# luxfi/tfhe

Hardware: AMD Instinct MI355X
Metric: PBS/sec at TFHE 128-bit default (N=1024), batch=4096; 1/2/4/8 MI355X (higher is better)
Workload: dtype f64

## Files before the change

tfhe_amd/csrc/pbs_fft.hip:

```cpp
#pragma clang fp contract(off)
#include <hip/hip_runtime.h>

#include <type_traits>

#include "fft512.h"
#include "gl64.h"
#include "ntt1024.h"
#include "pbs_kernels.h"

namespace tfhe {
namespace fftk {

__device__ __forceinline__ void fft_fwd_real(const double (&a)[16], double (&xr)[8], double (&xi)[8], double2* T,
                                             int lane, const double2* tw) {
#pragma unroll
  for (int e = 0; e < 8; e++) {
    xr[e] = a[e];
    xi[e] = a[e + 8];
  }
  dft512_fwd(xr, xi, T, lane, TBase(lane), tw);
}

__device__ __forceinline__ void fft_inv_real(double (&xr)[8], double (&xi)[8], double2* T, int lane, TBase tb,
                                             const double2* tw) {
  dft512_inv(xr, xi, T, lane, tb, tw);
  twist_slots<true>(xr, xi);
}

__device__ __forceinline__ int ms2048(u64 x) { return (int)((((x >> 52) + 1) >> 1) & 2047u); }

__device__ __forceinline__ u32 decomp_state(u64 x) { return ((u32)(x >> 32) + 1024u) >> 11; }
__device__ __forceinline__ int decomp_step(u32& st, u32 bmask) {
  const u32 b = __builtin_amdgcn_ubfe(st, 13, bmask);
  const u32 W = st + 63u + b;
  const u32 stn = W >> 7;
  int d;
  asm("v_mad_i32_i24 %0, %1, %2, %3" : "=v"(d) : "v"(stn), "s"(-128), "v"(st));
  st = stn;
  return d;
}
__device__ __forceinline__ u32 decomp_state_not(u64 S) { return (1023u - (u32)(S >> 32)) >> 11; }
__device__ __forceinline__ double decomp_top(u32 st) {
  int t;
  asm("v_bfe_i32 %0, %1, 0, 7" : "=v"(t) : "v"(0u - st));
  return -(double)t;
}

__device__ __forceinline__ void mac_first(double& re, double& im, double dr, double di, double2 k) {
  re = dr * k.x;
  re = __builtin_fma(-di, k.y, re);
  im = dr * k.y;
  im = __builtin_fma(di, k.x, im);
}
__device__ __forceinline__ void mac_next(double& re, double& im, double dr, double di, double2 k) {
  re = __builtin_fma(dr, k.x, re);
  re = __builtin_fma(-di, k.y, re);
  im = __builtin_fma(dr, k.y, im);
  im = __builtin_fma(di, k.x, im);
}

constexpr double BSK_SCALE = 0x1p-41;
__global__ __launch_bounds__(64) void bsk_to_fourier_kernel(const u64* __restrict__ bsk_std,
                                                            double2* __restrict__ bsk_f,
                                                            const double2* __restrict__ tw) {
  __shared__ __attribute__((aligned(16))) double2 T[T_C64];
  const int lane = threadIdx.x;
  const size_t q = blockIdx.x;
  const u64* src = bsk_std + q * N1K;
  double a[16], xr[8], xi[8];
#pragma unroll
  for (int e = 0; e < 16; e++) a[e] = i64_to_f64(src[64 * e + lane]);
  fft_fwd_real(a, xr, xi, T, lane, tw);
  const size_t j = q % 2, r = (q / 2) % 6, i = q / 12;
  double2* dst = bsk_f + ((i * 6 + (r / 3) * 3 + (2 - r % 3)) * 2 + j) * M;
#pragma unroll
  for (int e = 0; e < 8; e++) dst[64 * e + lane] = make_double2(xr[e] * BSK_SCALE, xi[e] * BSK_SCALE);
}

__global__ __launch_bounds__(64) void fft_fwd_kernel(const u64* __restrict__ in, double2* __restrict__ out,
                                                     const double2* __restrict__ tw) {
  __shared__ __attribute__((aligned(16))) double2 T[T_C64];
  const int lane = threadIdx.x;
  const u64* src = in + (size_t)blockIdx.x * N1K;
  double a[16], xr[8], xi[8];
#pragma unroll
  for (int e = 0; e < 16; e++) a[e] = i64_to_f64(src[64 * e + lane]);
  fft_fwd_real(a, xr, xi, T, lane, tw);
  double2* dst = out + (size_t)blockIdx.x * M;
#pragma unroll
  for (int e = 0; e < 8; e++) dst[64 * e + lane] = make_double2(xr[e], xi[e]);
}

__global__ __launch_bounds__(64) void fft_inv_kernel(const double2* __restrict__ in, double* __restrict__ out,
                                                     const double2* __restrict__ tw) {
  __shared__ __attribute__((aligned(16))) double2 T[T_C64];
  const int lane = threadIdx.x;
  const double2* src = in + (size_t)blockIdx.x * M;
  double xr[8], xi[8];
#pragma unroll
  for (int e = 0; e < 8; e++) {
    const double2 v = src[64 * e + lane];
    xr[e] = v.x;
    xi[e] = v.y;
  }
  fft_inv_real(xr, xi, T, lane, TBase(lane), tw);
  double* dst = out + (size_t)blockIdx.x * N1K;
#pragma unroll
  for (int e = 0; e < 8; e++) {
    dst[64 * e + lane] = xr[e];
    dst[64 * (e + 8) + lane] = xi[e];
  }
}

constexpr unsigned dispatch_half(unsigned wg, unsigned cus) { return wg / cus; }
constexpr bool wg_prio_hi(unsigned wg, unsigned cus) { return dispatch_half(wg, cus) & 1u; }
constexpr bool wg_staggered(unsigned wg, unsigned cus) { return dispatch_half(wg, cus) == 1u; }
namespace dh_check {
constexpr bool same_as_bit8(unsigned n) {
  for (unsigned w = 0; w < n; w++)
    if (wg_prio_hi(w, 256) != (((w >> 8) & 1u) != 0) || wg_staggered(w, 256) != (w < 512 && ((w >> 8) & 1u))) return false;
  return true;
}
static_assert(same_as_bit8(4096), "dispatch_half(., 256) must reproduce the 256-CU split");
static_assert(!wg_prio_hi(31, 32) && wg_prio_hi(32, 32) && wg_prio_hi(63, 32) && !wg_prio_hi(64, 32) && wg_prio_hi(96, 32), "32 CUs");
static_assert(!wg_staggered(31, 32) && wg_staggered(32, 32) && wg_staggered(63, 32) && !wg_staggered(64, 32) && !wg_staggered(96, 32), "32 CUs");
static_assert(!wg_prio_hi(303, 304) && wg_prio_hi(304, 304) && wg_prio_hi(607, 304) && !wg_prio_hi(608, 304) && wg_prio_hi(912, 304), "304 CUs");
static_assert(!wg_staggered(303, 304) && wg_staggered(304, 304) && wg_staggered(607, 304) && !wg_staggered(608, 304) && !wg_staggered(912, 304), "304 CUs");
}

constexpr int STEP_C64 = 4 * M;
template <int CTS>
struct FpShared {
  double2 twI[M];
  double2 K[1][STEP_C64];
  double2 T[2 * CTS][T_C64];
};
typedef __attribute__((address_space(3))) u64 lds_u64;

struct RotW {
  u32 wb;
  bool w15;
  __device__ __forceinline__ RotW(int a, int lane, double2* T)
      : wb((u32)(uintptr_t)(lds_u64*)&((u64*)T)[lane + (a & 63)]), w15(lane + (a & 63) >= 64) {}
};
template <int E>
__device__ __forceinline__ void rotation_store_pair(u64 v0, u64 v1, RotW w) {
  ((lds_u64*)(uintptr_t)w.wb)[64 * E] = v0;
  if constexpr (E < 14) {
    ((lds_u64*)(uintptr_t)w.wb)[64 * (E + 1)] = v1;
  } else {
    const u32 a15 = w.w15 ? w.wb + 960u * 8u - 8192u : w.wb + 960u * 8u;
    *(lds_u64*)(uintptr_t)a15 = w.w15 ? 0 - v1 : v1;
  }
}
__device__ __forceinline__ void rotation_store(const u64 (&v)[16], int a, int lane, double2* T) {
  const RotW w(a, lane, T);
  rotation_store_pair<0>(v[0], v[1], w);
  rotation_store_pair<2>(v[2], v[3], w);
  rotation_store_pair<4>(v[4], v[5], w);
  rotation_store_pair<6>(v[6], v[7], w);
  rotation_store_pair<8>(v[8], v[9], w);
  rotation_store_pair<10>(v[10], v[11], w);
  rotation_store_pair<12>(v[12], v[13], w);
  rotation_store_pair<14>(v[14], v[15], w);
}
__device__ __forceinline__ void rotation_states(const u64 (&v)[16], int a, int lane, double2* T, u32 (&st)[16]) {
  u64* Tu = (u64*)T;
  const int A = (a >> 6) & 15;
  const bool sgn = a >= 1024;
  const u32 rb = (u32)(uintptr_t)(lds_u64*)&Tu[lane] - 512u * (u32)A;
  const u32 wmask = (1u << A) - 1u;
  const u64 mbits = (u32)__builtin_amdgcn_readfirstlane(wmask ^ (sgn ? ~0u : 0u));
  u64 x[16];
  __builtin_amdgcn_fence(__ATOMIC_ACQ_REL, "wavefront");
  __builtin_amdgcn_sched_barrier(0);
#pragma unroll
  for (int e = 0; e < 16; e++)
    x[e] = ((const lds_u64*)(uintptr_t)(rb + (__builtin_amdgcn_ubfe(wmask, e, 1) << 13)))[64 * e];
  __builtin_amdgcn_sched_barrier(0);
#pragma unroll
  for (int e = 0; e < 16; e++) {
    u64 M;
    asm("s_bfe_i64 %0, %1, %2" : "=s"(M) : "s"(mbits), "i"(e | (1 << 16)));
    st[e] = decomp_state_not(~(x[e] ^ M) + (v[e] + M));
  }
  lds_order();
}

template <int C>
__device__ __forceinline__ void exchange_partials(const double (&o0r)[8], const double (&o0i)[8], const double (&o1r)[8],
                                                  const double (&o1i)[8], double (&xr)[8], double (&xi)[8], double2* T,
                                                  const double2* Tp, int lane) {
#pragma unroll
  for (int e = 0; e < 8; e++) {
    T[64 * e + lane] = C ? make_double2(o0r[e], o0i[e]) : make_double2(o1r[e], o1i[e]);
    xr[e] = C ? o1r[e] : o0r[e];
    xi[e] = C ? o1i[e] : o0i[e];
  }
  __syncthreads();
  double2 w[8];
  __builtin_amdgcn_sched_barrier(0);
#pragma unroll
  for (int e = 0; e < 8; e++) w[e] = Tp[64 * e + lane];
  __builtin_amdgcn_sched_barrier(0);
#pragma unroll
  for (int e = 0; e < 8; e++) {
    xr[e] = xr[e] + w[e].x;
    xi[e] = xi[e] + w[e].y;
  }
  __syncthreads();
}

template <int NW>
__device__ __forceinline__ void load_step_buf4(__amdgpu_buffer_rsrc_t bsr, int g, double2* dst, int wave_s, int voff) {
  static_assert((32 / NW) % 4 == 0 && 16 % (32 / NW) == 0, "groups of four blocks inside one component row");
  const int i = g / 3, q = g - 3 * (g / 3);
#pragma unroll
  for (int h = 0; h < 32 / NW; h += 4) {
    const int blk = wave_s * (32 / NW) + h;
    const int c = blk >> 4;
    const int soff = ((i * 6 + c * 3 + q) * (2 * M)) * (int)sizeof(double2) + (blk & 15) * 1024;
    auto* ld = (__attribute__((address_space(3))) void*)((char*)dst + blk * 1024);
    __builtin_amdgcn_raw_ptr_buffer_load_lds(bsr, ld, 16, voff, soff, 0, 0);
    __builtin_amdgcn_raw_ptr_buffer_load_lds(bsr, ld, 16, voff, soff, 1024, 0);
    __builtin_amdgcn_raw_ptr_buffer_load_lds(bsr, ld, 16, voff, soff, 2048, 0);
    __builtin_amdgcn_raw_ptr_buffer_load_lds(bsr, ld, 16, voff, soff, 3072, 0);
  }
}

#ifndef FFT_DMASTAMP
#define FFT_DMASTAMP 0
#endif
#if FFT_DMASTAMP
__device__ unsigned long long g_dmast[64 * 4 * 4];
#endif

#ifndef FFT_WGTIME
#define FFT_WGTIME 0
#endif
#if FFT_WGTIME
__device__ unsigned long long g_wgt[4 * 16384];
#endif
template <int CTS, bool WRITE_ACC, bool WRITE_BIG>
__global__ __launch_bounds__(128 * CTS, 4 / CTS) void blind_rotate_fft_pair_kernel(
    const u64* __restrict__ lwe_in, int n, size_t B, const u64* __restrict__ luts, const u32* __restrict__ lut_index,
    int n_lut, const double2* __restrict__ bsk, const double2* __restrict__ tw_g, u64* __restrict__ out_big,
    u64* __restrict__ out_acc, int n_cus) {
  constexpr int NW = 2 * CTS;
  __shared__ __attribute__((aligned(16))) FpShared<CTS> sh;
#if FFT_WGTIME
  const unsigned long long wg_t0 = __builtin_amdgcn_s_memrealtime();
#endif
  const int wave = threadIdx.x >> 6, lane = threadIdx.x & 63;
  const int c = wave & 1;
  const size_t b_raw = (size_t)blockIdx.x * CTS + (wave >> 1);
  const bool live = b_raw < B;
  const size_t b = live ? b_raw : B - 1;
  const u64* ct = lwe_in + b * (size_t)(n + 1);
  double2* T = sh.T[wave];
  const double2* Tp = sh.T[wave ^ 1];
  const int wave_s = __builtin_amdgcn_readfirstlane(wave);
  const int c_s = wave_s & 1;

  const __amdgpu_buffer_rsrc_t bsr =
      __builtin_amdgcn_make_buffer_rsrc((void*)bsk, (short)0, n * 6 * 2 * M * (int)sizeof(double2), 0x00020000);
  const int voff = lane * 16;
  for (int q = threadIdx.x; q < M; q += 64 * NW) sh.twI[q] = tw_g[TW_I + q];

  u64 acc[16];
  {
    int li = lut_index ? (int)lut_index[b] : 0;
    li = (li < 0 || li >= n_lut) ? 0 : li;
    const u64* lut = luts + (size_t)li * N1K;
    const int s = (2048 - ms2048(ct[n])) & 2047;
#pragma unroll
    for (int e = 0; e < 16; e++) {
      int d = 64 * e + lane - s;
      bool neg = false;
      if (d < 0) { d += N1K; neg = !neg; }
      if (d < 0) { d += N1K; neg = !neg; }
      const u64 v = gl_to_torus(lut[d]);
      acc[e] = c ? (neg ? 0 - v : v) : 0;
    }
  }

  const TBase tb(lane);
  const double2* twA = tw_g + TW_A;
  const double2* twI = sh.twI;
  const double2* twB = twA + M;
  double2 wa[8];
  __syncthreads();
#pragma unroll
  for (int e = 0; e < 8; e++) wa[e] = twA[64 * e + lane];
  double2 wb[8];
#pragma unroll
  for (int e = 1; e < 8; e++) wb[e] = twB[64 * e + lane];
  wb[0] = make_double2(1.0, 0.0);
  const bool prio_hi = wg_prio_hi(blockIdx.x, (unsigned)n_cus);
  const unsigned prio_flag = __builtin_amdgcn_readfirstlane(prio_hi ? 1u : 0u);
  auto base_prio = [&]() {
    asm volatile(
        "s_cmp_lg_u32 %0, 0\n\ts_cbranch_scc0 .Lbp0_%=\n\ts_setprio 1\n\ts_branch .Lbp1_%=\n"
        ".Lbp0_%=:\n\ts_setprio 0\n.Lbp1_%=:" ::"s"(prio_flag) : "scc");
  };
  base_prio();
  if (wg_staggered(blockIdx.x, (unsigned)n_cus)) __builtin_amdgcn_s_sleep(127);
#if FFT_DMASTAMP
  unsigned long long dma_cyc[3] = {0, 0, 0};
  const unsigned long long loop_t0 = __builtin_amdgcn_s_memtime();
#endif
  auto ms2048_hi = [](u32 hi) { return (int)((((hi >> 20) + 1u) >> 1) & 2047u); };
  const u32* ct_hi = (const u32*)ct + 1;
  int a_s = __builtin_amdgcn_readfirstlane(ms2048_hi(ct_hi[0]));
  rotation_store(acc, a_s, lane, T);
  for (int i = 0; i < n; i++) {
    u32 st[16];
    rotation_states(acc, a_s, lane, T, st);
    u32 ct_next = ct_hi[2 * (size_t)(i + 1)];
    double o0r[8], o0i[8], o1r[8], o1i[8];
    auto level = [&](auto qc) {
      constexpr int q = decltype(qc)::value;
      const int g = 3 * i + q;
      if (q > 0) base_prio();
      if (q > 0) __syncthreads();
#if FFT_DMASTAMP
      __builtin_amdgcn_sched_barrier(0);
      const unsigned long long dma_t0 = __builtin_amdgcn_s_memtime();
#endif
      load_step_buf4<NW>(bsr, g, sh.K[0], wave_s, voff);
#if FFT_DMASTAMP
      dma_cyc[q] += __builtin_amdgcn_s_memtime() - dma_t0;
      __builtin_amdgcn_sched_barrier(0);
#endif
      double xr[8], xi[8];
#pragma unroll
      for (int e = 0; e < 8; e++) {
        if constexpr (q == 2) {
          xr[e] = decomp_top(st[e]);
          xi[e] = decomp_top(st[e + 8]);
        } else {
          xr[e] = (double)decomp_step(st[e], 1u);
          xi[e] = (double)decomp_step(st[e + 8], 1u);
        }
      }
      dft512_fwd_rab_p(xr, xi, T, lane, tb, wa, wb);
      glds_barrier();
      if constexpr (q == 0) {
        asm volatile("" : "+v"(ct_next));
        a_s = ms2048_hi(__builtin_amdgcn_readfirstlane(ct_next));
      }
      __builtin_amdgcn_s_setprio(3);
      const double2* k0 = sh.K[0] + c * (2 * M) + lane;
      const double2* k1 = k0 + M;
      if constexpr (q > 0) {
        constexpr int D = q == 2 ? 2 : 1;
        double2 ku[8], kv[8];
#pragma unroll
        for (int e = 0; e < D; e++) {
          ku[e] = k0[64 * e];
          kv[e] = k1[64 * e];
        }
#pragma unroll
        for (int e = 0; e < 8; e++) {
          if (e + D < 8) {
            ku[e + D] = k0[64 * (e + D)];
            kv[e + D] = k1[64 * (e + D)];
          }
          __builtin_amdgcn_sched_barrier(0);
          mac_next(o0r[e], o0i[e], xr[e], xi[e], ku[e]);
          mac_next(o1r[e], o1i[e], xr[e], xi[e], kv[e]);
          __builtin_amdgcn_sched_barrier(0);
        }
        return;
      }
#pragma unroll
      for (int e = 0; e < 8; e++) {
        const double2 u = k0[64 * e], v = k1[64 * e];
        if constexpr (q == 0) {
          mac_first(o0r[e], o0i[e], xr[e], xi[e], u);
          mac_first(o1r[e], o1i[e], xr[e], xi[e], v);
        } else {
          mac_next(o0r[e], o0i[e], xr[e], xi[e], u);
          mac_next(o1r[e], o1i[e], xr[e], xi[e], v);
        }
      }
    };
    level(std::integral_constant<int, 0>{});
    level(std::integral_constant<int, 1>{});
    level(std::integral_constant<int, 2>{});
    base_prio();
    double xr[8], xi[8];
    if (c_s) exchange_partials<1>(o0r, o0i, o1r, o1i, xr, xi, T, Tp, lane);
    else exchange_partials<0>(o0r, o0i, o1r, o1i, xr, xi, T, Tp, lane);
    dft512_inv_rb_p(xr, xi, T, lane, tb, wb, twI);
    twist_slots<true>(xr, xi);
    {
      const RotW w(a_s, lane, T);
      auto upd = [&](auto ec) {
        constexpr int e = decltype(ec)::value;
        acc[e] = torus_acc_add_y(acc[e], e < 8 ? xr[e & 7] : xi[e & 7]);
        acc[e + 1] = torus_acc_add_y(acc[e + 1], e < 8 ? xr[(e + 1) & 7] : xi[(e + 1) & 7]);
        rotation_store_pair<e>(acc[e], acc[e + 1], w);
        __builtin_amdgcn_sched_barrier(0);
      };
      __builtin_amdgcn_sched_barrier(0);
      upd(std::integral_constant<int, 0>{});
      upd(std::integral_constant<int, 2>{});
      upd(std::integral_constant<int, 4>{});
      upd(std::integral_constant<int, 6>{});
      upd(std::integral_constant<int, 8>{});
      upd(std::integral_constant<int, 10>{});
      upd(std::integral_constant<int, 12>{});
      upd(std::integral_constant<int, 14>{});
    }
  }
#if FFT_DMASTAMP
  if (lane == 0 && blockIdx.x < 64 && wave < 4) {
    unsigned long long* o = g_dmast + (blockIdx.x * 4 + wave) * 4;
    o[0] = dma_cyc[0];
    o[1] = dma_cyc[1];
    o[2] = dma_cyc[2];
    o[3] = __builtin_amdgcn_s_memtime() - loop_t0;
  }
#endif
#if FFT_WGTIME
  if (threadIdx.x == 0 && blockIdx.x < 16384) {
    const unsigned long long t1 = __builtin_amdgcn_s_memrealtime();
    g_wgt[4 * blockIdx.x] = wg_t0;
    g_wgt[4 * blockIdx.x + 1] = t1;
    g_wgt[4 * blockIdx.x + 2] = (unsigned)__builtin_amdgcn_s_getreg(4 | (31 << 11));
    g_wgt[4 * blockIdx.x + 3] = (unsigned)__builtin_amdgcn_s_getreg(20 | (31 << 11));
  }
#endif

  if (!live) return;
  if (WRITE_ACC) {
    u64* oa = out_acc + b * 2048 + c * N1K;
#pragma unroll
    for (int e = 0; e < 16; e++) oa[64 * e + lane] = acc[e];
  }
  if (WRITE_BIG) {
    u64* ob = out_big + b * (size_t)(N1K + 1);
    if (c == 0) {
#pragma unroll
      for (int e = 0; e < 16; e++) {
        const int idx = 64 * e + lane;
        if (idx == 0) ob[0] = acc[e];
        else ob[N1K - idx] = 0 - acc[e];
      }
    } else if (lane == 0) {
      ob[N1K] = acc[0];
    }
  }
}

constexpr int FL_THREADS = 512;
constexpr int FL_MAXN = 1024;
struct FftLatShared {
  double2 tw[TW_C64];
  u64 A[2][N1K];
  double2 F[6][M];
  double2 T[6][T_C64];
  unsigned short ab[FL_MAXN];
};

__device__ __forceinline__ void lat_load_key(const double2* __restrict__ bsk, int i, int j, int s0, int lane,
                                             double2 (&kv)[6][2]) {
#pragma unroll
  for (int r = 0; r < 6; r++)
#pragma unroll
    for (int t = 0; t < 2; t++) kv[r][t] = bsk[((size_t)(i * 6 + r) * 2 + j) * M + 64 * (s0 + t) + lane];
}

__device__ __forceinline__ void lat_barrier() {
  asm volatile("s_waitcnt lgkmcnt(0)\n\ts_barrier" ::: "memory");
}

#ifndef FFT_LATSTAMP
#define FFT_LATSTAMP 0
#endif
#if FFT_LATSTAMP
struct LatStamp {
  unsigned long long acc[6] = {0, 0, 0, 0, 0, 0}, t0 = 0;
  __device__ __forceinline__ void start() { t0 = __builtin_amdgcn_s_memrealtime(); }
  __device__ __forceinline__ void mark(int k) { acc[k] += __builtin_amdgcn_s_memrealtime() - t0; }
};
__device__ unsigned long long g_latst[8 * 8 * 6];
#define LS_START(st) st.start()
#define LS_MARK(st, k) st.mark(k)
#else
struct LatStamp {};
#define LS_START(st)
#define LS_MARK(st, k)
#endif
__device__ __forceinline__ void lat_cmux(FftLatShared& sh, const u64* __restrict__ ct, int i, int wave, int lane,
                                         TBase tb, int j, int s0, const double2 (&kv)[6][2], LatStamp& ls) {
  LS_START(ls);
  const int a = i < FL_MAXN ? (int)sh.ab[i] : ms2048(ct[i]);
  if (wave < 6) {
    const int c = wave / 3, q = wave % 3;
    const u64* acc = sh.A[c];
    u32 st[16];
#pragma unroll
    for (int e = 0; e < 16; e++) {
      const int t = 64 * e + lane - a + 2 * N1K;
      const u64 x = acc[t & (N1K - 1)];
      const u64 r = (t & N1K) ? 0 - x : x;
      st[e] = decomp_state(r - acc[64 * e + lane]);
    }
    int dg[16];
    for (int qq = 0; qq <= q; qq++) {
      const u32 bmask = qq < 2 ? 1u : 0u;
#pragma unroll
      for (int e = 0; e < 16; e++) dg[e] = decomp_step(st[e], bmask);
    }
    double xr[8], xi[8];
#pragma unroll
    for (int e = 0; e < 8; e++) {
      xr[e] = (double)dg[e];
      xi[e] = (double)dg[e + 8];
    }
    dft512_fwd(xr, xi, sh.T[wave], lane, tb, sh.tw);
#pragma unroll
    for (int e = 0; e < 8; e++) sh.F[wave][64 * e + lane] = make_double2(xr[e], xi[e]);
  }
  LS_MARK(ls, 0);
  lat_barrier();
  LS_MARK(ls, 1);
  {
    double2* O = sh.T[2 + j];
#pragma unroll
    for (int t = 0; t < 2; t++) {
      const int e = s0 + t;
      double re[2], im[2];
#pragma unroll
      for (int r = 0; r < 6; r++) {
        const double2 D = sh.F[r][64 * e + lane], K = kv[r][t];
        const int cc = r / 3;
        if (r % 3 == 0) mac_first(re[cc], im[cc], D.x, D.y, K);
        else mac_next(re[cc], im[cc], D.x, D.y, K);
      }
      O[64 * e + lane] = make_double2(re[0] + re[1], im[0] + im[1]);
    }
  }
  LS_MARK(ls, 2);
  lat_barrier();
  LS_MARK(ls, 3);
  if (wave < 2) {
    const double2* O = sh.T[2 + wave];
    double xr[8], xi[8];
#pragma unroll
    for (int e = 0; e < 8; e++) {
      const double2 v = O[64 * e + lane];
      xr[e] = v.x;
      xi[e] = v.y;
    }
    fft_inv_real(xr, xi, sh.T[wave], lane, tb, sh.tw);
    u64* acc = sh.A[wave];
#pragma unroll
    for (int e = 0; e < 8; e++) {
      acc[64 * e + lane] = torus_acc_add_y(acc[64 * e + lane], xr[e]);
      acc[64 * (e + 8) + lane] = torus_acc_add_y(acc[64 * (e + 8) + lane], xi[e]);
    }
  }
  LS_MARK(ls, 4);
  lat_barrier();
  LS_MARK(ls, 5);
}

template <bool WRITE_ACC, bool WRITE_BIG>
__global__ __launch_bounds__(FL_THREADS, 1) void blind_rotate_fft_lat_kernel(
    const u64* __restrict__ lwe_in, int n, size_t B, const u64* __restrict__ luts, const u32* __restrict__ lut_index,
    int n_lut, const double2* __restrict__ bsk, const double2* __restrict__ tw_g, u64* __restrict__ out_big,
    u64* __restrict__ out_acc) {
  __shared__ __attribute__((aligned(16))) FftLatShared sh;
  const int wave = threadIdx.x >> 6, lane = threadIdx.x & 63;
  const size_t b = blockIdx.x;
  const u64* ct = lwe_in + b * (size_t)(n + 1);
  const TBase tb(lane);

  for (int q = threadIdx.x; q < TW_C64; q += FL_THREADS) sh.tw[q] = tw_g[q];
  for (int q = threadIdx.x; q < n && q < FL_MAXN; q += FL_THREADS) sh.ab[q] = (unsigned short)ms2048(ct[q]);
  {
    int li = lut_index ? (int)lut_index[b] : 0;
    li = (li < 0 || li >= n_lut) ? 0 : li;
    const u64* lut = luts + (size_t)li * N1K;
    const int s = (2048 - ms2048(ct[n])) & 2047;
    for (int q = threadIdx.x; q < N1K; q += FL_THREADS) {
      int d = q - s;
      bool neg = false;
      if (d < 0) { d += N1K; neg = !neg; }
      if (d < 0) { d += N1K; neg = !neg; }
      const u64 v = gl_to_torus(lut[d]);
      sh.A[0][q] = 0;
      sh.A[1][q] = neg ? 0 - v : v;
    }
  }
  __syncthreads();

  const int j = wave >> 2, s0 = (wave & 3) * 2;
  LatStamp ls;
  double2 kva[6][2], kvb[6][2];
  lat_load_key(bsk, 0, j, s0, lane, kva);
  for (int i = 0; i < n; i += 2) {
    if (i + 1 < n) lat_load_key(bsk, i + 1, j, s0, lane, kvb);
    lat_cmux(sh, ct, i, wave, lane, tb, j, s0, kva, ls);
    if (i + 1 >= n) break;
    if (i + 2 < n) lat_load_key(bsk, i + 2, j, s0, lane, kva);
    lat_cmux(sh, ct, i + 1, wave, lane, tb, j, s0, kvb, ls);
  }

#if FFT_LATSTAMP
  if (lane == 0 && b < 8)
    for (int k = 0; k < 6; k++) g_latst[(b * 8 + wave) * 6 + k] = ls.acc[k];
#endif
  if (WRITE_ACC) {
    u64* oa = out_acc + b * 2048;
    for (int q = threadIdx.x; q < 2 * N1K; q += FL_THREADS) oa[q] = sh.A[q >> 10][q & (N1K - 1)];
  }
  if (WRITE_BIG) {
    u64* ob = out_big + b * (size_t)(N1K + 1);
    for (int q = threadIdx.x; q <= N1K; q += FL_THREADS)
      ob[q] = q == N1K ? sh.A[1][0] : q == 0 ? sh.A[0][0] : 0 - sh.A[0][N1K - q];
  }
}

static double fs_sin(double x) {
  double x2 = x * x, term = x, sum = 0.0;
  for (int i = 1; i <= 21; i += 2) { sum += term; term = -term * x2 / (double)((i + 1) * (i + 2)); }
  return sum;
}
static double fs_cos(double x) {
  double x2 = x * x, term = 1.0, sum = 0.0;
  for (int i = 0; i <= 20; i += 2) { sum += term; term = -term * x2 / (double)((i + 1) * (i + 2)); }
  return sum;
}
static void tw_octant(uint32_t t, uint32_t m, double* c, double* s) {
  const double x = (double)t * (6.28318530717958647692 / (double)m);
  *c = fs_cos(x);
  *s = fs_sin(x);
}
static void tw_quarter(uint32_t t, uint32_t m, double* c, double* s) {
  if (8 * t > m) {
    double cu, su;
    tw_octant(m / 4 - t, m, &cu, &su);
    *c = su;
    *s = cu;
  } else {
    tw_octant(t, m, c, s);
  }
}
static void twiddle(uint32_t t, uint32_t m, double* c, double* s) {
  t %= m;
  bool neg = false;
  if (2 * t > m) { t = m - t; neg = true; }
  double cc, ss;
  if (4 * t > m) {
    double cu, su;
    tw_quarter(t - m / 4, m, &cu, &su);
    cc = -su;
    ss = cu;
  } else {
    tw_quarter(t, m, &cc, &ss);
  }
  *c = cc;
  *s = neg ? -ss : ss;
}

}

void fft_twiddle(uint32_t t, uint32_t m, double* c, double* s) { fftk::twiddle(t, m, c, s); }

static bool make_tables_f1k(u64* tw) {
  using namespace fftk;
  double* t = (double*)tw;
  for (uint32_t j = 0; j < (uint32_t)M; j++) twiddle(j, 4 * M, &t[2 * (TW_TWIST + j)], &t[2 * (TW_TWIST + j) + 1]);
  for (uint32_t e = 0; e < 8; e++)
    for (uint32_t L = 0; L < 64; L++) {
      twiddle((L * (1 + 4 * e)) % (4 * M), 4 * M, &t[2 * (TW_A + 64 * e + L)], &t[2 * (TW_A + 64 * e + L) + 1]);
      twiddle((8 * (L & 7) * e) % M, M, &t[2 * (TW_B + 64 * e + L)], &t[2 * (TW_B + 64 * e + L) + 1]);
      twiddle((((L & 7) + 8 * e) * (4 * (L >> 3) + 1)) % (4 * M), 4 * M, &t[2 * (TW_I + 64 * e + L)],
              &t[2 * (TW_I + 64 * e + L) + 1]);
    }
  for (int e = 0; e < 8; e++) {
    double c, s, c2, s2;
    twiddle(64u * e, 2048u, &c, &s);
    twiddle(128u * e, 4096u, &c2, &s2);
    if (c != ctw::SLOT[e].x || s != ctw::SLOT[e].y || c2 != c || s2 != s) return false;
  }
  return true;
}

static hipError_t convert_bsk_f1k(const u64* bsk_std, u64* bsk_f, size_t polys, const u64* tw, hipStream_t s) {
  if (polys == 0) return hipSuccess;
  hipLaunchKernelGGL(fftk::bsk_to_fourier_kernel, dim3((unsigned)polys), dim3(64), 0, s, bsk_std, (double2*)bsk_f,
                     (const double2*)tw);
  return hipGetLastError();
}

static hipError_t blind_rotate_f1k(const u64* lwe_in, size_t B, int n, const u64* luts, const u32* lut_index,
                                   int n_lut, const u64* bsk_f, const u64* tw, u64* out_big, u64* out_acc,
                                   bool latency, int n_cus, hipStream_t s) {
  using namespace fftk;
  if (B == 0) return hipSuccess;
  if (n_cus <= 0) n_cus = 256;
  const double2 *bk = (const double2*)bsk_f, *t = (const double2*)tw;
  if (latency)
    return launch_out_mode(out_acc, out_big, [&](auto wa, auto wb) {
      hipLaunchKernelGGL((blind_rotate_fft_lat_kernel<wa(), wb()>), dim3((unsigned)B), dim3(FL_THREADS), 0, s, lwe_in,
                         n, B, luts, lut_index, n_lut, bk, t, out_big, out_acc);
    });
  constexpr int CTS = 2;
  return launch_out_mode(out_acc, out_big, [&](auto wa, auto wb) {
    hipLaunchKernelGGL((blind_rotate_fft_pair_kernel<CTS, wa(), wb()>), dim3((unsigned)((B + CTS - 1) / CTS)),
                       dim3(128 * CTS), 0, s, lwe_in, n, B, luts, lut_index, n_lut, bk, t, out_big, out_acc, n_cus);
  });
}

#if FFT_LATSTAMP
extern "C" int tfhe_hip_debug_latstamps(unsigned long long* out, size_t n) {
  if (n > 8 * 8 * 6) n = 8 * 8 * 6;
  return hipMemcpyFromSymbol(out, HIP_SYMBOL(fftk::g_latst), n * 8, 0, hipMemcpyDeviceToHost) == hipSuccess ? 0 : -1;
}
#endif
#if FFT_DMASTAMP
extern "C" int tfhe_hip_debug_dmastamps(unsigned long long* out, size_t n) {
  if (n > 64 * 4 * 4) n = 64 * 4 * 4;
  return hipMemcpyFromSymbol(out, HIP_SYMBOL(fftk::g_dmast), n * 8, 0, hipMemcpyDeviceToHost) == hipSuccess ? 0 : -1;
}
#endif
#if FFT_WGTIME
extern "C" int tfhe_hip_debug_wgtimes(unsigned long long* out, size_t n) {
  if (n > 4 * 16384) n = 4 * 16384;
  return hipMemcpyFromSymbol(out, HIP_SYMBOL(fftk::g_wgt), n * 8, 0, hipMemcpyDeviceToHost) == hipSuccess ? 0 : -1;
}
#endif

static hipError_t fft_fwd_f1k(const u64* in, size_t count, u64* out, const u64* tw, hipStream_t s) {
  if (count == 0) return hipSuccess;
  hipLaunchKernelGGL(fftk::fft_fwd_kernel, dim3((unsigned)count), dim3(64), 0, s, in, (double2*)out,
                     (const double2*)tw);
  return hipGetLastError();
}

static hipError_t fft_inv_f1k(const u64* in, size_t count, u64* out, const u64* tw, hipStream_t s) {
  if (count == 0) return hipSuccess;
  hipLaunchKernelGGL(fftk::fft_inv_kernel, dim3((unsigned)count), dim3(64), 0, s, (const double2*)in, (double*)out,
                     (const double2*)tw);
  return hipGetLastError();
}

#ifndef __HIP_DEVICE_COMPILE__
const br_engine ENGINE_FFT1K = {true,
                                N1K,
                                256,
                                "blind_rotate_fft_lat_kernel",
                                "blind_rotate_fft_pair_kernel",
                                2 * fftk::TW_C64,
                                make_tables_f1k,
                                convert_bsk_f1k,
                                blind_rotate_f1k,
                                fft_fwd_f1k,
                                fft_inv_f1k};
#endif

}
```

Measured before the change: 190,300.

## Load level-0 bootstrap keys directly to registers and prefetch level-1 keys early

Level 0 of each blind-rotation step now pulls its key coefficients straight from global memory into registers with buffer loads, split around the decomposition. This drops the LDS DMA and the barrier that level 0 used to need. The level-1 LDS DMA is issued right after level 0's multiply-accumulate, which overlaps it with compute and removes one __syncthreads per iteration. The epilogue also recomputes lane and batch indices from scalar or mbcnt values, and asm fences keep voff live, both to ease register pressure. The cost is more VGPRs for the sixteen in-flight key registers, plus a possible risk to LDS reuse ordering with fewer barriers.

```diff
diff --git a/tfhe_amd/csrc/pbs_fft.hip b/tfhe_amd/csrc/pbs_fft.hip
--- a/tfhe_amd/csrc/pbs_fft.hip
+++ b/tfhe_amd/csrc/pbs_fft.hip
@@ -228,6 +228,19 @@
   }
 }
 
+typedef unsigned int u32x4 __attribute__((ext_vector_type(4)));
+template <int E0, int E1>
+__device__ __forceinline__ void load_step0_keys(__amdgpu_buffer_rsrc_t bsr, int i, int c_s, int voff, double2 (&ku)[8],
+                                                double2 (&kv)[8]) {
+  const int soff = ((i * 6 + c_s * 3) * (2 * M)) * (int)sizeof(double2);
+#pragma unroll
+  for (int e = E0; e < E1; e++) {
+    const int so = soff + (e >> 2) * 4096, vo = voff + (e & 3) * 1024;
+    ku[e] = __builtin_bit_cast(double2, __builtin_amdgcn_raw_buffer_load_b128(bsr, vo, so, 0));
+    kv[e] = __builtin_bit_cast(double2, __builtin_amdgcn_raw_buffer_load_b128(bsr, vo, so + M * (int)sizeof(double2), 0));
+  }
+}
+
 #ifndef FFT_DMASTAMP
 #define FFT_DMASTAMP 0
 #endif
@@ -251,7 +264,8 @@
 #if FFT_WGTIME
   const unsigned long long wg_t0 = __builtin_amdgcn_s_memrealtime();
 #endif
-  const int wave = threadIdx.x >> 6, lane = threadIdx.x & 63;
+  const int wave = threadIdx.x >> 6;
+  int lane = threadIdx.x & 63;
   const int c = wave & 1;
   const size_t b_raw = (size_t)blockIdx.x * CTS + (wave >> 1);
   const bool live = b_raw < B;
@@ -264,7 +278,7 @@
 
   const __amdgpu_buffer_rsrc_t bsr =
       __builtin_amdgcn_make_buffer_rsrc((void*)bsk, (short)0, n * 6 * 2 * M * (int)sizeof(double2), 0x00020000);
-  const int voff = lane * 16;
+  int voff = lane * 16;
   for (int q = threadIdx.x; q < M; q += 64 * NW) sh.twI[q] = tw_g[TW_I + q];
 
   u64 acc[16];
@@ -316,18 +330,26 @@
   for (int i = 0; i < n; i++) {
     u32 st[16];
     rotation_states(acc, a_s, lane, T, st);
+    asm volatile("" : "+v"(voff));
     u32 ct_next = ct_hi[2 * (size_t)(i + 1)];
     double o0r[8], o0i[8], o1r[8], o1i[8];
     auto level = [&](auto qc) {
       constexpr int q = decltype(qc)::value;
       const int g = 3 * i + q;
       if (q > 0) base_prio();
-      if (q > 0) __syncthreads();
+      if (q == 1) __builtin_amdgcn_sched_barrier(0);
+      if (q == 2) __syncthreads();
+      double2 ku0[8], kv0[8];
+      if constexpr (q == 0) {
+        __builtin_amdgcn_sched_barrier(0);
+        load_step0_keys<0, 4>(bsr, i, c_s, voff, ku0, kv0);
+        __builtin_amdgcn_sched_barrier(0);
+      }
 #if FFT_DMASTAMP
       __builtin_amdgcn_sched_barrier(0);
       const unsigned long long dma_t0 = __builtin_amdgcn_s_memtime();
 #endif
-      load_step_buf4<NW>(bsr, g, sh.K[0], wave_s, voff);
+      if (q == 2) load_step_buf4<NW>(bsr, g, sh.K[0], wave_s, voff);
 #if FFT_DMASTAMP
       dma_cyc[q] += __builtin_amdgcn_s_memtime() - dma_t0;
       __builtin_amdgcn_sched_barrier(0);
@@ -343,46 +365,53 @@
           xi[e] = (double)decomp_step(st[e + 8], 1u);
         }
       }
+      if constexpr (q == 0) {
+        __builtin_amdgcn_sched_barrier(0);
+        load_step0_keys<4, 8>(bsr, i, c_s, voff, ku0, kv0);
+        __builtin_amdgcn_sched_barrier(0);
+      }
       dft512_fwd_rab_p(xr, xi, T, lane, tb, wa, wb);
-      glds_barrier();
       if constexpr (q == 0) {
         asm volatile("" : "+v"(ct_next));
         a_s = ms2048_hi(__builtin_amdgcn_readfirstlane(ct_next));
+        __builtin_amdgcn_s_setprio(3);
+#pragma unroll
+        for (int e = 0; e < 8; e++) {
+          mac_first(o0r[e], o0i[e], xr[e], xi[e], ku0[e]);
+          mac_first(o1r[e], o1i[e], xr[e], xi[e], kv0[e]);
+        }
+        __builtin_amdgcn_sched_barrier(0);
+#if FFT_DMASTAMP
+        const unsigned long long dma_t1 = __builtin_amdgcn_s_memtime();
+#endif
+        load_step_buf4<NW>(bsr, g + 1, sh.K[0], wave_s, voff);
+#if FFT_DMASTAMP
+        dma_cyc[1] += __builtin_amdgcn_s_memtime() - dma_t1;
+#endif
+        __builtin_amdgcn_sched_barrier(0);
+        return;
       }
+      glds_barrier();
       __builtin_amdgcn_s_setprio(3);
       const double2* k0 = sh.K[0] + c * (2 * M) + lane;
       const double2* k1 = k0 + M;
-      if constexpr (q > 0) {
-        constexpr int D = q == 2 ? 2 : 1;
-        double2 ku[8], kv[8];
-#pragma unroll
-        for (int e = 0; e < D; e++) {
-          ku[e] = k0[64 * e];
-          kv[e] = k1[64 * e];
+      constexpr int D = q == 2 ? 2 : 1;
+      double2 ku[8], kv[8];
+#pragma unroll
+      for (int e = 0; e < D; e++) {
+        ku[e] = k0[64 * e];
+        kv[e] = k1[64 * e];
+      }
+#pragma unroll
+      for (int e = 0; e < 8; e++) {
+        if (e + D < 8) {
+          ku[e + D] = k0[64 * (e + D)];
+          kv[e + D] = k1[64 * (e + D)];
         }
-#pragma unroll
-        for (int e = 0; e < 8; e++) {
-          if (e + D < 8) {
-            ku[e + D] = k0[64 * (e + D)];
-            kv[e + D] = k1[64 * (e + D)];
-          }
-          __builtin_amdgcn_sched_barrier(0);
-          mac_next(o0r[e], o0i[e], xr[e], xi[e], ku[e]);
-          mac_next(o1r[e], o1i[e], xr[e], xi[e], kv[e]);
-          __builtin_amdgcn_sched_barrier(0);
-        }
-        return;
-      }
-#pragma unroll
-      for (int e = 0; e < 8; e++) {
-        const double2 u = k0[64 * e], v = k1[64 * e];
-        if constexpr (q == 0) {
-          mac_first(o0r[e], o0i[e], xr[e], xi[e], u);
-          mac_first(o1r[e], o1i[e], xr[e], xi[e], v);
-        } else {
-          mac_next(o0r[e], o0i[e], xr[e], xi[e], u);
-          mac_next(o1r[e], o1i[e], xr[e], xi[e], v);
-        }
+        __builtin_amdgcn_sched_barrier(0);
+        mac_next(o0r[e], o0i[e], xr[e], xi[e], ku[e]);
+        mac_next(o1r[e], o1i[e], xr[e], xi[e], kv[e]);
+        __builtin_amdgcn_sched_barrier(0);
       }
     };
     level(std::integral_constant<int, 0>{});
@@ -434,14 +463,21 @@
 #endif
 
   if (!live) return;
+  const size_t bo = (size_t)blockIdx.x * CTS + (size_t)(wave_s >> 1);
+  const int co = c_s;
+  {
+    u32 z;
+    asm volatile("v_mov_b32 %0, 0" : "=v"(z));
+    lane = (int)__builtin_amdgcn_mbcnt_hi(~0u, __builtin_amdgcn_mbcnt_lo(~0u, z));
+  }
   if (WRITE_ACC) {
-    u64* oa = out_acc + b * 2048 + c * N1K;
+    u64* oa = out_acc + bo * 2048 + co * N1K;
 #pragma unroll
     for (int e = 0; e < 16; e++) oa[64 * e + lane] = acc[e];
   }
   if (WRITE_BIG) {
-    u64* ob = out_big + b * (size_t)(N1K + 1);
-    if (c == 0) {
+    u64* ob = out_big + bo * (size_t)(N1K + 1);
+    if (co == 0) {
 #pragma unroll
       for (int e = 0; e < 16; e++) {
         const int idx = 64 * e + lane;
```

Measured after the change: 193,000 (median of 6 runs). 1.01x the previous value.
